# aayush9400/3D-Condtional-Stable-Diffusion

Hardware: AMD Instinct MI355X
Metric: latent volumes/sec at 32^3x8ch T=1000 DDPM (higher is better)
Workload: dtype f32 (f16 hi+lo x3 MFMA, f32 accumulate)

## Files before the change

### 3d-condtional-stable-diffusion_amd/csrc/dm3d_conv_h3w.hip

```cpp
#include <cstdlib>
#include "dm3d_conv_h3v2_parts.h"

using namespace h3v2;

#ifdef DM3D_CLOCK_STAMPS
__device__ unsigned long long* g_dbg_stamps_w = nullptr;
extern "C" int dm3d_debug_set_stamps_wino(void* p) { return (int)hipMemcpyToSymbol(HIP_SYMBOL(g_dbg_stamps_w), &p, sizeof(p)); }
#ifndef STAMP_MASK
#define STAMP_MASK 0xffffffffu
#endif
#define STAMP(i) do { if (((STAMP_MASK >> (i)) & 1u) && g_dbg_stamps_w && wave == 0 && __builtin_amdgcn_mbcnt_lo(~0u, 0u) == 0u && cur.ntile == 0 && cur.khalf == 0 && item / ny < 4096u) { \
    g_dbg_stamps_w[(item / ny) * 32 + (i)] = __builtin_amdgcn_s_memtime(); \
    if ((i) == 1) g_dbg_stamps_w[(item / ny) * 32 + 30] = __builtin_amdgcn_s_memrealtime(); \
    if ((i) == 28) g_dbg_stamps_w[(item / ny) * 32 + 31] = __builtin_amdgcn_s_memrealtime(); } } while (0)
#else
#define STAMP(i) do { } while (0)
#endif

namespace {

template <int N, int I = 0, class F>
__device__ __forceinline__ void static_for(F&& f) {
    if constexpr (I < N) {
        f(std::integral_constant<int, I>{});
        static_for<N, I + 1>(f);
    }
}

constexpr int pass_of(int s) { return 3 * s - (s + 1) / 5; }

template <int MODE>
__global__ __launch_bounds__(256, 1) void conv3d_igemm_h3w(const ConvArgs p) {
    constexpr int TD = 8, TH = 8, TW = 8, CK = 16, NT = 64, NW = 4;
    constexpr int HD = TD + 2, HH = TH + 2, HROWS = HD * HH;
    constexpr int RREC = 17;
    constexpr int NS = 20;
    constexpr int WPAIR = 2 * NT * REC;
    constexpr int RING = 4;
    constexpr int WSLOT = WPAIR * 2 / 1024 / NW;
    constexpr int NLD = 5;
    constexpr bool pro = MODE == 1, xh2 = MODE == 2;
    constexpr int PLOADS = pro ? 4 : 0;

    extern __shared__ __attribute__((aligned(16))) _Float16 smem_w[];
    _Float16* lds_w = smem_w;
    _Float16* lds_in = smem_w + RING * WPAIR;

    const int tid = threadIdx.x;
    const int lane = tid & 63, wave = __builtin_amdgcn_readfirstlane(tid >> 6);

    const int ntiles = p.coutpad / NT;
    const unsigned ny = (unsigned)(ntiles * p.ksplit);
    const int bpv = p.bd * p.bh * p.bw;
    const int cpp = p.nchunks / p.ksplit;
    unsigned item, item_end, item_step;
    {
        const unsigned n_items = (unsigned)(p.batch * bpv) * ny, G = gridDim.x, d = blockIdx.x;
        if ((G & 7u) == 0 && (n_items & 7u) == 0) {
            const unsigned per = n_items >> 3;
            item = (d & 7u) * per + (d >> 3); item_end = (d & 7u) * per + per; item_step = G >> 3;
        } else { item = d; item_end = n_items; item_step = G; }
    }
    struct Item { int b, oz0, oy0, ox0, ntile, khalf; };
    auto decode = [&](unsigned w) {
        Item it;
        unsigned brick = w / ny;
        const unsigned by = w - brick * ny;
        it.ntile = (int)(by % (unsigned)ntiles); it.khalf = (int)(by / (unsigned)ntiles);
        it.b = (int)(brick / (unsigned)bpv);
        brick -= (unsigned)(it.b * bpv);
        it.oz0 = (int)(brick / (unsigned)(p.bh * p.bw)) * TD;
        it.oy0 = (int)((brick / (unsigned)p.bw) % (unsigned)p.bh) * TH;
        it.ox0 = (int)(brick % (unsigned)p.bw) * TW;
        it.b = __builtin_amdgcn_readfirstlane(it.b); it.oz0 = __builtin_amdgcn_readfirstlane(it.oz0); it.oy0 = __builtin_amdgcn_readfirstlane(it.oy0);
        it.ox0 = __builtin_amdgcn_readfirstlane(it.ox0); it.ntile = __builtin_amdgcn_readfirstlane(it.ntile); it.khalf = __builtin_amdgcn_readfirstlane(it.khalf);
        return it;
    };
    Item cur = decode(item);
    auto vec_row = [&](const Item& it) { return p.vec ? (p.vec_idx ? p.vec_idx[it.b] : it.b) : 0; };
    int vrow_s = vec_row(cur);
    int c_lo = cur.khalf * cpp, c_hi = c_lo + cpp;
    STAMP(0);

    int piece = 0;
    bool s_act = false;
    unsigned st_addr = 0u, a_pair[2] = {0u, 0u}, wb_hi = 0u;
    int w_voff = 0;
    constexpr int DZB = HH * RREC * REC * 2, DYB = RREC * REC * 2;
    const unsigned in_addr = (unsigned)(size_t)(__attribute__((address_space(3))) _Float16*)lds_in;
    const unsigned w_addr = (unsigned)(size_t)(__attribute__((address_space(3))) _Float16*)lds_w;
    auto lane_setup = [&]() {
        int t = tid;
        asm volatile("" : "+v"(t));
        const int ln = t & 63, half = ln >> 5, q = (ln >> 4) & 1, row = ln & 15;
        piece = t & 1;
        s_act = (t >> 1) < HROWS;
        const int srow = s_act ? (t >> 1) : HROWS - 1;
        st_addr = in_addr + (unsigned)(srow * RREC * REC + ((piece ^ ((srow % HH) & 2)) << 3)) * 2u;
        const int ay = row & 3, xq = (row >> 2) ^ (row >> 3);
        const unsigned a_base = in_addr + (unsigned)((((2 * wave) * HH + ay) * RREC + xq) * (REC * 2));
        unsigned sl[3];
#pragma unroll
        for (int dy = 0; dy < 3; ++dy) sl[dy] = (unsigned)((q ^ ((ay + dy) & 2)) << 4);
        a_pair[0] = a_base + (half ? DYB + sl[1] : sl[0]);
        a_pair[1] = a_base + 2 * DYB + sl[2] + (half ? DZB : 0);
        const int b_pos = pi_pos(row);
        wb_hi = w_addr + (unsigned)((half * NT + b_pos) * REC + ((q ^ swz(b_pos)) << 3)) * 2u;
        w_voff = wave * 1024 + ln * 16;
    };
    lane_setup();
    int sb, gv0;
    bool row_in, x_lo, x_hi;
    auto stage_setup = [&](const Item& it) {
        int tid_s = tid;
        asm volatile("" : "+v"(tid_s));
        const int sr = (tid_s >> 1) < HROWS ? (tid_s >> 1) : HROWS - 1, hz = sr / HH, hy = sr % HH;
        const int iz = it.oz0 - 1 + hz, iy = it.oy0 - 1 + hy;
        row_in = iz >= 0 && iz < p.ind && iy >= 0 && iy < p.inh;
        x_lo = it.ox0 > 0; x_hi = it.ox0 + TW < p.inw;
        const int izc = iz < 0 ? 0 : (iz >= p.ind ? p.ind - 1 : iz), iyc = iy < 0 ? 0 : (iy >= p.inh ? p.inh - 1 : iy);
        gv0 = ((it.b * p.ind + izc) * p.inh + iyc) * p.inw + it.ox0 - 1;
        sb = it.b;
    };
    stage_setup(cur);
    f32x4v acc[4][4][4];

    const auto w_rsrc = __builtin_amdgcn_make_buffer_rsrc(const_cast<void*>(p.wpk), (short)0, (int)((long)ntiles * p.nchunks * (NS * WPAIR * 2)), 0x00020000);
    auto w_chunk = [&](int ntile_, int ch_) { return (unsigned)((ntile_ * p.nchunks + ch_) * (NS * WPAIR * 2)); };
    unsigned w_cur = w_chunk(cur.ntile, c_lo), w_nxt = w_cur;
    auto fetch_w1 = [&](const unsigned off, int slot, const int i) {
        char* dst = reinterpret_cast<char*>(lds_w) + slot * (WPAIR * 2) + wave * 1024;
        __builtin_amdgcn_raw_ptr_buffer_load_lds(w_rsrc, (__attribute__((address_space(3))) void*)(dst + i * (NW * 1024)), 16, w_voff,
                                                 (int)(off + i * (NW * 1024)), 0, 0);
    };
#pragma unroll
    for (int i = 0; i < RING; ++i) { fetch_w1(w_cur + i * (WPAIR * 2), i, 0); fetch_w1(w_cur + i * (WPAIR * 2), i, 1); }

    f32x4 va[10][2];
    u32x4 oh[4], ol[4];
    u32x4 o3h[4], o3l[4];
    f32x4 sc0 = {1.f, 1.f, 1.f, 1.f}, sc1 = sc0, sh0 = {0.f, 0.f, 0.f, 0.f}, sh1 = sh0;
    bool km[3][2] = {{true, true}, {true, true}, {true, true}};
    bool ok0 = true, ok1 = true;
    auto load_voxel = [&](int ch, int hx) {
        const int hxc = hx == 0 ? (x_lo ? 0 : 1) : (hx == 9 ? (x_hi ? 9 : 8) : hx);
        const unsigned gv = (unsigned)(gv0 + hxc);
        if (xh2) {
            const char* base = reinterpret_cast<const char*>(p.x1) + (size_t)ch * 64;
            const unsigned off = gv * ((unsigned)p.c1 * 4u) + (unsigned)piece * 16u;
            va[hx][0] = *reinterpret_cast<const f32x4*>(base + off);
            va[hx][1] = *reinterpret_cast<const f32x4*>(base + off + 32u);
            return;
        }
        const int c0 = ch * CK;
        const float* src;
        int ldc, cb;
        if (c0 < p.c1) { src = p.x1; ldc = p.c1; cb = c0; } else { src = p.x2; ldc = p.c2; cb = c0 - p.c1; }
        const int cpos = cb + piece * 8;
        const int off0 = cpos < ldc ? cpos : 0, off1 = cpos + 4 < ldc ? cpos + 4 : 0;
        const char* base = reinterpret_cast<const char*>(src);
        const unsigned voff = gv * ((unsigned)ldc * 4u);
        va[hx][0] = *reinterpret_cast<const f32x4*>(base + (voff + (unsigned)off0 * 4u));
        va[hx][1] = *reinterpret_cast<const f32x4*>(base + (voff + (unsigned)off1 * 4u));
    };
    auto load_chunk_params = [&](int ch) {
        if (xh2) return;
        const int c0 = ch * CK;
        const int ldc = c0 < p.c1 ? p.c1 : p.c2, cpos = (c0 < p.c1 ? c0 : c0 - p.c1) + piece * 8;
        ok0 = cpos < ldc;
        ok1 = cpos + 4 < ldc;
        if (pro) {
            const int s0 = ok0 ? c0 + piece * 8 : 0, s1 = ok1 ? c0 + piece * 8 + 4 : 0;
            const size_t bo = (size_t)sb * p.pro_bstride;
            sc0 = *reinterpret_cast<const f32x4*>(p.pscale + bo + s0);
            sh0 = *reinterpret_cast<const f32x4*>(p.pshift + bo + s0);
            sc1 = *reinterpret_cast<const f32x4*>(p.pscale + bo + s1);
            sh1 = *reinterpret_cast<const f32x4*>(p.pshift + bo + s1);
        }
    };
    auto halo_ops = [&](int s) {
        if (s < 0) s += NS;
        if (s >= NLD) return 0;
        return 4 + (s == 0 ? PLOADS : 0);
    };
    typedef float f32x2 __attribute__((ext_vector_type(2)));
    h8 g_hi, g_lo;
#define DM3D_PIN(x) asm volatile("" :: "v"(x))
    auto act_quad = [&](const int hx, const int h) {
        const int col = hx == 0 ? 0 : (hx == 9 ? 2 : 1);
        f32x4 v;
        if (xh2) {
            if (h == 0) { g_hi = __builtin_bit_cast(h8, va[hx][0]); g_lo = __builtin_bit_cast(h8, va[hx][1]); }
#pragma unroll
            for (int e = 0; e < 4; ++e) { const _Float16 a = g_hi[4 * h + e], b = g_lo[4 * h + e]; v[e] = (float)a + (float)b; }
            if (!km[col][0]) v = f32x4{0.f, 0.f, 0.f, 0.f};
        } else {
            v = va[hx][h];
            if (pro) {
                const f32x4 y = __builtin_elementwise_fma(v, h ? sc1 : sc0, h ? sh1 : sh0);
                const f32x4 z = y * -1.4426950408889634f;
                f32x4 d;
#pragma unroll
                for (int e = 0; e < 4; ++e) d[e] = __builtin_amdgcn_exp2f(z[e]);
                d = d + 1.0f;
#pragma unroll
                for (int e = 0; e < 4; ++e) d[e] = __builtin_amdgcn_rcpf(d[e]);
                v = y * d;
            }
            if (!km[col][h]) v = f32x4{0.f, 0.f, 0.f, 0.f};
        }
        DM3D_PIN(v);
        va[hx][h] = v;
    };
    auto split_pair = [&](const int t, const int xt, const int j) {
        const int h = j >> 1, c = 2 * (j & 1);
        auto d = [&](const int k) { return f32x2{va[2 * xt + k][h][c], va[2 * xt + k][h][c + 1]}; };
        const f32x2 x = t == 0 ? d(0) - d(2) : (t == 1 ? d(1) + d(2) : (t == 2 ? d(2) - d(1) : d(1) - d(3)));
        const float x0 = x[0], x1 = x[1];
        unsigned int a, r;
        float r0, r1;
        asm volatile("v_cvt_pk_f16_f32 %0, %4, %5\n\tv_fma_mix_f32 %2, %0, -1.0, %4 op_sel_hi:[1,0,0]\n\t"
                     "v_fma_mix_f32 %3, %0, -1.0, %5 op_sel:[1,0,0] op_sel_hi:[1,0,0]\n\tv_cvt_pk_f16_f32 %1, %2, %3"
                     : "=&v"(a), "=&v"(r), "=&v"(r0), "=&v"(r1) : "v"(x0), "v"(x1));
        if (t == 3) { o3h[xt][j] = a; o3l[xt][j] = r; } else { oh[xt][j] = a; ol[xt][j] = r; }
    };
    auto chunk_masks = [&]() {
        km[0][0] = row_in && x_lo && ok0; km[0][1] = row_in && x_lo && ok1; km[1][0] = row_in && ok0; km[1][1] = row_in && ok1;
        km[2][0] = row_in && x_hi && ok0; km[2][1] = row_in && x_hi && ok1;
    };
    auto store_record = [&](const int t, const int xt) {
        if (s_act) {
            unsigned lo_addr;
            const u32x4 dh = t == 3 ? o3h[xt] : oh[xt], dl = t == 3 ? o3l[xt] : ol[xt];
            switch (t * 4 + xt) {
#define DM3D_ST(k_) case k_: asm volatile("ds_write_b128 %1, %2 offset:%4\n\tv_xor_b32 %0, 32, %1\n\tds_write_b128 %0, %3 offset:%4" \
                                          : "=&v"(lo_addr) : "v"(st_addr), "v"(dh), "v"(dl), "n"((k_) * REC * 2) : "memory"); break;
                DM3D_ST(0) DM3D_ST(1) DM3D_ST(2) DM3D_ST(3) DM3D_ST(4) DM3D_ST(5) DM3D_ST(6) DM3D_ST(7)
                DM3D_ST(8) DM3D_ST(9) DM3D_ST(10) DM3D_ST(11) DM3D_ST(12) DM3D_ST(13) DM3D_ST(14) DM3D_ST(15)
#undef DM3D_ST
            }
        }
    };
    auto lds_barrier = [&]() {
        asm volatile("s_waitcnt lgkmcnt(0)" ::: "memory");
        __builtin_amdgcn_s_barrier();
        asm volatile("" ::: "memory");
    };

#pragma unroll
    for (int hx = 0; hx < 10; ++hx) load_voxel(c_lo, hx);
    load_chunk_params(c_lo);
#pragma unroll
    for (int t = 0; t < 4; ++t)
#pragma unroll
        for (int pi = 0; pi < 4; ++pi)
#pragma unroll
            for (int ni = 0; ni < 4; ++ni) {
                acc[t][pi][ni] = f32x4v{0.f, 0.f, 0.f, 0.f};
                asm volatile("" : "+a"(acc[t][pi][ni]));
            }
    __builtin_amdgcn_s_waitcnt(0x0F70);
    chunk_masks();
#pragma unroll
    for (int hx = 0; hx < 10; ++hx) { act_quad(hx, 0); act_quad(hx, 1); }
#pragma unroll
    for (int t = 0; t < 4; ++t) {
#pragma unroll
        for (int u = 0; u < 16; ++u) split_pair(t, u >> 2, u & 3);
#pragma unroll
        for (int xt = 0; xt < 4; ++xt) store_record(t, xt);
    }
    lds_barrier();

    h8 ah[4], al[4], bh[4], bl[4];
    auto lo_of = [](const unsigned a) { unsigned r; asm volatile("v_xor_b32 %0, 32, %1" : "=v"(r) : "v"(a)); return r; };
#define DM3D_DSR(dst, addr, off) asm volatile("ds_read_b128 %0, %1 offset:%2" : "=v"(dst) : "v"(addr), "n"(off))
    constexpr int GOFF = 4 * RREC * REC * 2, SOFF = HH * RREC * REC * 2;
    auto a_hi = [&](const int s) { return a_pair[(s % 5) >= 3]; };
    auto read_a = [&](h8 (&dst)[4], const int s, const int i, const unsigned a0) {
        const int tp = s % 5;
        switch (((s / 5) * 4 + i) * 3 + (tp < 3 ? tp : tp - 3)) {
#define DM3D_RA1(t_, i_, z_) case ((t_) * 4 + (i_)) * 3 + (z_): DM3D_DSR(dst[i_], a0, (z_) * DZB + (t_) * 4 * REC * 2 + ((i_) >> 1) * SOFF + ((i_) & 1) * GOFF); break;
#define DM3D_RA(t_, i_) DM3D_RA1(t_, i_, 0) DM3D_RA1(t_, i_, 1) DM3D_RA1(t_, i_, 2)
            DM3D_RA(0, 0) DM3D_RA(0, 1) DM3D_RA(0, 2) DM3D_RA(0, 3) DM3D_RA(1, 0) DM3D_RA(1, 1) DM3D_RA(1, 2) DM3D_RA(1, 3)
            DM3D_RA(2, 0) DM3D_RA(2, 1) DM3D_RA(2, 2) DM3D_RA(2, 3) DM3D_RA(3, 0) DM3D_RA(3, 1) DM3D_RA(3, 2) DM3D_RA(3, 3)
#undef DM3D_RA
#undef DM3D_RA1
        }
    };
    auto read_b = [&](h8 (&dst)[4], const int slot, const int i, const unsigned wa) {
        switch (slot * 4 + i) {
#define DM3D_RB(k_, i_) case (k_) * 4 + (i_): DM3D_DSR(dst[i_], wa, (k_) * WPAIR * 2 + (i_) * 16 * REC * 2); break;
            DM3D_RB(0, 0) DM3D_RB(0, 1) DM3D_RB(0, 2) DM3D_RB(0, 3) DM3D_RB(1, 0) DM3D_RB(1, 1) DM3D_RB(1, 2) DM3D_RB(1, 3)
            DM3D_RB(2, 0) DM3D_RB(2, 1) DM3D_RB(2, 2) DM3D_RB(2, 3) DM3D_RB(3, 0) DM3D_RB(3, 1) DM3D_RB(3, 2) DM3D_RB(3, 3)
#undef DM3D_RB
        }
    };
    f32x4 g_y, g_z;
    float g_x0 = 0.f, g_x1 = 0.f, g_r0 = 0.f;
    unsigned int g_a = 0u;
    constexpr int NPASS = 3 * NS - NS / 5;
    auto stores_at_head = [&](int p) {
        p = (p + NPASS) % NPASS;
        if (p == 36 || p == 37 || p == 39 || p == 40 || p == 42 || p == 43) return 2;
        if (p == 38 || p == 41 || p == 44) return 4;
        return p == 54 ? 8 : 0;
    };
    auto head_stores = [&](const int p) {
        if (p == 36) store_record(0, 0); else if (p == 37) store_record(0, 1); else if (p == 38) { store_record(0, 2); store_record(0, 3); }
        else if (p == 39) store_record(1, 0); else if (p == 40) store_record(1, 1); else if (p == 41) { store_record(1, 2); store_record(1, 3); }
        else if (p == 42) store_record(2, 0); else if (p == 43) store_record(2, 1); else if (p == 44) { store_record(2, 2); store_record(2, 3); }
        else if (p == 54) {
#pragma unroll
            for (int xt = 0; xt < 4; ++xt) store_record(3, xt);
        }
    };
    auto slot_gap = [&](const int G) {
        if (G == 191) { chunk_masks(); return; }
        if (G >= 192 && G < 552) {
            const int i = (G - 192) / 18, r = (G - 192) % 18;
            const int hx = i >> 1, h = i & 1, col = hx == 0 ? 0 : (hx == 9 ? 2 : 1);
            if (xh2) {
                auto mix = [&](const int c) {
                    float d;
                    const float hv = va[hx][0][c >> 1], lv = va[hx][1][c >> 1];
                    if (c & 1) asm volatile("v_fma_mix_f32 %0, %1, 1.0, %2 op_sel:[1,0,1] op_sel_hi:[1,0,1]" : "=v"(d) : "v"(hv), "v"(lv));
                    else asm volatile("v_fma_mix_f32 %0, %1, 1.0, %2 op_sel:[0,0,0] op_sel_hi:[1,0,1]" : "=v"(d) : "v"(hv), "v"(lv));
                    return d;
                };
                if (h == 0) {
                    if (r < 2) { g_y[2 * r] = mix(2 * r); g_y[2 * r + 1] = mix(2 * r + 1); }
                } else {
                    if (r < 2) {
                        const float v0 = mix(4 + 2 * r), v1 = mix(5 + 2 * r);
                        va[hx][1][2 * r] = v0; va[hx][1][2 * r + 1] = v1;
                    } else if (r < 4) {
                        const int c = 2 * (r - 2);
                        float v0 = km[col][0] ? g_y[c] : 0.0f, v1 = km[col][0] ? g_y[c + 1] : 0.0f;
                        DM3D_PIN(v0); DM3D_PIN(v1);
                        va[hx][0][c] = v0; va[hx][0][c + 1] = v1;
                    } else if (r < 6) {
                        const int c = 2 * (r - 4);
                        float v0 = km[col][0] ? va[hx][1][c] : 0.0f, v1 = km[col][0] ? va[hx][1][c + 1] : 0.0f;
                        DM3D_PIN(v0); DM3D_PIN(v1);
                        va[hx][1][c] = v0; va[hx][1][c + 1] = v1;
                    }
                }
                return;
            }
            if (!pro) {
                if (r < 2) {
                    const int c = 2 * r;
                    float v0 = km[col][h] ? va[hx][h][c] : 0.0f, v1 = km[col][h] ? va[hx][h][c + 1] : 0.0f;
                    DM3D_PIN(v0); DM3D_PIN(v1);
                    va[hx][h][c] = v0; va[hx][h][c + 1] = v1;
                }
                return;
            }
            const f32x4 sc = h ? sc1 : sc0, sh = h ? sh1 : sh0;
            if (r < 2) {
                const int c = 2 * r;
                g_y[c] = fmaf(va[hx][h][c], sc[c], sh[c]); g_y[c + 1] = fmaf(va[hx][h][c + 1], sc[c + 1], sh[c + 1]);
                DM3D_PIN(g_y[c]); DM3D_PIN(g_y[c + 1]);
            } else if (r < 4) {
                const int c = 2 * (r - 2);
                g_z[c] = g_y[c] * -1.4426950408889634f; g_z[c + 1] = g_y[c + 1] * -1.4426950408889634f;
                DM3D_PIN(g_z[c]); DM3D_PIN(g_z[c + 1]);
            } else if (r < 8) {
                g_z[r - 4] = __builtin_amdgcn_exp2f(g_z[r - 4]);
                DM3D_PIN(g_z[r - 4]);
            } else if (r < 10) {
                const int c = 2 * (r - 8);
                g_z[c] = 1.0f + g_z[c]; g_z[c + 1] = 1.0f + g_z[c + 1];
                DM3D_PIN(g_z[c]); DM3D_PIN(g_z[c + 1]);
            } else if (r < 14) {
                g_z[r - 10] = __builtin_amdgcn_rcpf(g_z[r - 10]);
                DM3D_PIN(g_z[r - 10]);
            } else if (r < 16) {
                const int c = 2 * (r - 14);
                g_y[c] = g_y[c] * g_z[c]; g_y[c + 1] = g_y[c + 1] * g_z[c + 1];
                DM3D_PIN(g_y[c]); DM3D_PIN(g_y[c + 1]);
            } else {
                const int c = 2 * (r - 16);
                float v0 = km[col][h] ? g_y[c] : 0.0f, v1 = km[col][h] ? g_y[c + 1] : 0.0f;
                DM3D_PIN(v0); DM3D_PIN(v1);
                va[hx][h][c] = v0; va[hx][h][c + 1] = v1;
            }
            return;
        }
        if ((G >= 560 && G < 704) || (G >= 816 && G < 864)) {
            const int t = G < 608 ? 0 : (G < 656 ? 1 : (G < 704 ? 2 : 3));
            const int q = G - (t == 0 ? 560 : (t == 1 ? 608 : (t == 2 ? 656 : 816)));
            const int u = q / 3, st = q % 3, xt = u >> 2, j = u & 3, h = j >> 1, c = 2 * (j & 1);
            if (st == 0) {
                auto d = [&](const int k, const int e) { return va[2 * xt + k][h][c + e]; };
                g_x0 = t == 0 ? d(0, 0) - d(2, 0) : (t == 1 ? d(1, 0) + d(2, 0) : (t == 2 ? d(2, 0) - d(1, 0) : d(1, 0) - d(3, 0)));
                g_x1 = t == 0 ? d(0, 1) - d(2, 1) : (t == 1 ? d(1, 1) + d(2, 1) : (t == 2 ? d(2, 1) - d(1, 1) : d(1, 1) - d(3, 1)));
                DM3D_PIN(g_x0); DM3D_PIN(g_x1);
            } else if (st == 1) {
                asm volatile("v_cvt_pk_f16_f32 %0, %2, %3\n\tv_fma_mix_f32 %1, %0, -1.0, %2 op_sel_hi:[1,0,0]" : "=&v"(g_a), "=&v"(g_r0) : "v"(g_x0), "v"(g_x1));
            } else {
                unsigned int r;
                float r1;
                asm volatile("v_fma_mix_f32 %1, %2, -1.0, %3 op_sel:[1,0,0] op_sel_hi:[1,0,0]\n\tv_cvt_pk_f16_f32 %0, %4, %1" : "=&v"(r), "=&v"(r1) : "v"(g_a), "v"(g_x1), "v"(g_r0));
                if (t == 3) { o3h[xt][j] = g_a; o3l[xt][j] = r; } else { oh[xt][j] = g_a; ol[xt][j] = r; }
            }
        }
    };
#define DM3D_MFMA(T, PI, NI, A, B) asm volatile("v_mfma_f32_16x16x32_f16 %0, %1, %2, %0" : "+a"(acc[T][PI][NI]) : "v"(A[PI]), "v"(B[NI]))
#define DM3D_WAIT_LGKM(n) asm volatile("s_waitcnt lgkmcnt(%0)" :: "n"(n) : "memory")

    bool has_next = item + item_step < item_end;
    for (;;) {
    lane_setup();
    {
        const unsigned a_lo0 = lo_of(a_hi(0));
        read_a(al, 0, 0, a_lo0); read_a(al, 0, 1, a_lo0); read_a(al, 0, 2, a_lo0); read_a(al, 0, 3, a_lo0);
    }
    read_b(bh, 0, 0, wb_hi); read_b(bh, 0, 1, wb_hi); read_b(bh, 0, 2, wb_hi); read_b(bh, 0, 3, wb_hi);
    read_a(ah, 0, 0, a_hi(0)); read_a(ah, 0, 1, a_hi(0)); read_a(ah, 0, 2, a_hi(0)); read_a(ah, 0, 3, a_hi(0));
    STAMP(1);

    for (int ch = c_lo; ch < c_hi; ++ch) {
        asm volatile("" : "+v"(gv0));
        int ch_next;
        if (ch + 1 < c_hi) { ch_next = ch + 1; w_nxt = w_cur + NS * WPAIR * 2; }
        else if (has_next) {
            const Item n = decode(item + item_step);
            stage_setup(n); ch_next = n.khalf * cpp; w_nxt = w_chunk(n.ntile, ch_next);
        }
        else { ch_next = ch; w_nxt = w_cur; }
        static_for<NS>([&](auto S_) {
            constexpr int s = decltype(S_)::value, sn = (s + 1) % NS;
            constexpr int t = s / 5, ws = s & (RING - 1), ws1 = (s + 1) & (RING - 1);
            constexpr bool pad = s % 5 == 3, pre_pad = s % 5 == 2, post_pad = s % 5 == 4;
            constexpr int E = pass_of(s);
            constexpr bool swapped = (((s + 1) / 5) & 1) != 0;
            h8 (&fh)[4] = swapped ? al : ah;
            h8 (&fl)[4] = swapped ? ah : al;
            h8 (&fl_n)[4] = pad ? fh : fl;
            h8 (&fh_n)[4] = pad ? fl : fh;
            {
                constexpr int n_out = pad ? 0 : 4;
                switch (post_pad ? 0 : stores_at_head(E - 1)) {
                case 0: DM3D_WAIT_LGKM(n_out); break;
                case 2: DM3D_WAIT_LGKM(n_out + 2); break;
                case 4: DM3D_WAIT_LGKM(n_out + 4); break;
                default: DM3D_WAIT_LGKM(n_out + 8); break;
                }
            }
            head_stores(E);
            __builtin_amdgcn_sched_barrier(0);
            unsigned b_lo = 0u, a_lo = 0u;
#pragma unroll
            for (int g = 0; g < 16; ++g) {
                DM3D_MFMA(t, g >> 2, g & 3, fl, bh);
                slot_gap(16 * E + g);
                if (g == 2) b_lo = lo_of(wb_hi);
                if (g == 3) { read_b(bl, ws, 0, b_lo); read_b(bl, ws, 1, b_lo); }
                if (pre_pad) {
                    if (g == 4) asm volatile("v_subrev_u32 %0, %2, %1" : "=v"(a_lo) : "v"(a_pair[1]), "n"(DZB));
                    if (g == 5) asm volatile("v_xor_b32 %0, 32, %0" : "+v"(a_lo));
                    if (g == 6) asm volatile("v_cndmask_b32_e64 %0, %1, %0, %2" : "+v"(a_lo) : "v"(a_pair[1]), "s"(0xffffffff00000000ull));
                } else if (g == 6) a_lo = lo_of(a_hi(sn));
                if (g == 7) { read_b(bl, ws, 2, b_lo); read_b(bl, ws, 3, b_lo); read_a(fl_n, sn, 0, a_lo); }
                if (g == 11) { read_a(fl_n, sn, 1, a_lo); read_a(fl_n, sn, 2, a_lo); }
                if (g == 15) read_a(fl_n, sn, 3, a_lo);
                __builtin_amdgcn_sched_barrier(0);
            }
            {
                constexpr int DMA_BEHIND = 2 * WSLOT;
                const int extra = halo_ops(s - 3) + halo_ops(s - 2) + halo_ops(s - 1);
#define DM3D_WAIT_VM_LGKM4(n) __builtin_amdgcn_s_waitcnt((((n) & 15) | (7 << 4) | (4 << 8) | ((((n) >> 4) & 3) << 14)))
                switch (extra) {
                case 0:  DM3D_WAIT_VM_LGKM4(DMA_BEHIND); break;
                case 4:  DM3D_WAIT_VM_LGKM4(DMA_BEHIND + 4); break;
                case 8:  DM3D_WAIT_VM_LGKM4(DMA_BEHIND + 8); break;
                case 12: DM3D_WAIT_VM_LGKM4(DMA_BEHIND + 12); break;
                case 16: DM3D_WAIT_VM_LGKM4(DMA_BEHIND + 16); break;
                default: DM3D_WAIT_VM_LGKM4(0); break;
                }
#undef DM3D_WAIT_VM_LGKM4
                __builtin_amdgcn_s_barrier();
                asm volatile("" ::: "memory");
            }
            __builtin_amdgcn_sched_barrier(0);
            const unsigned w_src = s + RING < NS ? w_cur + (s + RING) * (WPAIR * 2) : w_nxt + (s + RING - NS) * (WPAIR * 2);
            fetch_w1(w_src, ws, 0);
            head_stores(E + 1);
            __builtin_amdgcn_sched_barrier(0);
#pragma unroll
            for (int g = 0; g < 16; ++g) {
                if (pad) {
                    DM3D_MFMA(t, g >> 2, g & 3, fl, bl);
                    slot_gap(16 * (E + 1) + g);
                    if (g == 2) { read_b(bh, ws1, 0, wb_hi); read_b(bh, ws1, 1, wb_hi); }
                    if (g == 3) { read_b(bh, ws1, 2, wb_hi); read_b(bh, ws1, 3, wb_hi); }
                    if (g == 4) read_a(fh_n, sn, 0, a_hi(sn));
                    if (g == 7 || g == 11 || g == 15) read_a(fh_n, sn, g >> 2, a_hi(sn));
                } else {
                    DM3D_MFMA(t, g & 3, g >> 2, fh, bh);
                    slot_gap(16 * (E + 1) + g);
                    if ((g & 3) == 3) read_b(bh, ws1, g >> 2, wb_hi);
                }
                if (g == 1) fetch_w1(w_src, ws, 1);
                if (s < NLD && g == 5) load_voxel(ch_next, 2 * s);
                if (s < NLD && g == 9) load_voxel(ch_next, 2 * s + 1);
                if (s == 0 && g == 13) load_chunk_params(ch_next);
                __builtin_amdgcn_sched_barrier(0);
            }
            if constexpr (!pad) {
                head_stores(E + 2);
                __builtin_amdgcn_sched_barrier(0);
#pragma unroll
                for (int g = 0; g < 16; ++g) {
                    DM3D_MFMA(t, g >> 2, g & 3, fh, bl);
                    slot_gap(16 * (E + 2) + g);
                    if (!pre_pad && (g & 3) == 3) read_a(fh, sn, g >> 2, a_hi(sn));
                    __builtin_amdgcn_sched_barrier(0);
                }
            }
        });
        w_cur = w_nxt;
    }
#undef DM3D_MFMA
#undef DM3D_WAIT_LGKM
#undef DM3D_PIN
#undef DM3D_DSR
    STAMP(28);
    const Brick br = {cur.b, cur.oz0, cur.oy0, cur.ox0, p.ooz, p.ooy, p.oox, cur.ntile, cur.khalf};
    {
        asm volatile("s_waitcnt lgkmcnt(0)" ::: "memory");
        STAMP(20);
        const bool skip = p.s_npairs > 0;
        if (skip) {
#pragma unroll
            for (int pi = 0; pi < 4; ++pi)
#pragma unroll
                for (int ni = 0; ni < 4; ++ni) {
                    const f32x4v m0 = acc[0][pi][ni], m1 = acc[1][pi][ni], m2 = acc[2][pi][ni], m3 = acc[3][pi][ni];
                    acc[0][pi][ni] = (m0 + m1) + m2;
                    acc[1][pi][ni] = (m1 - m2) - m3;
                    asm volatile("" : "+a"(acc[0][pi][ni]), "+a"(acc[1][pi][ni]));
                }
            const int p_lo = p.s_npairs * cur.khalf / p.ksplit, np = p.s_npairs * (cur.khalf + 1) / p.ksplit;
            int lane_t = lane;
            asm volatile("" : "+v"(lane_t));
            const int kq = lane_t >> 4, lhalf = kq >> 1, cq = (kq & 1) * 8, row_t = lane_t & 15;
            unsigned sv[8];
#pragma unroll
            for (int t = 0; t < 8; ++t) {
                const int z = 2 * wave + (t >> 2), y = 4 * ((t >> 1) & 1) + (row_t & 3), x = 2 * ((row_t >> 2) ^ (row_t >> 3)) + (t & 1);
                sv[t] = (unsigned)(((cur.b * p.ind + cur.oz0 + z) * p.inh + cur.oy0 + y) * p.inw + cur.ox0 + x);
            }
            const char* swf = reinterpret_cast<const char*>(p.swpk_f) + (size_t)cur.ntile * p.s_npairs * 8192 + lane_t * 16;
            f32x4 ar0[2][8], ar1[2][8];
            h8 bw[2][8];
            float lim0[2], lim1[2];
            auto t_load = [&](auto SET, int pp) {
                constexpr int S = decltype(SET)::value;
                const int c0 = (pp * 2 + lhalf) * CK;
                const float* src;
                int ldc, cb;
                if (c0 < p.sc1) { src = p.sx1; ldc = p.sc1; cb = c0; } else { src = p.sx2; ldc = p.sc2; cb = c0 - p.sc1; }
                const int cpos = cb + cq;
                const bool real = src != nullptr && cb < ldc && pp < np;
                const bool k0 = real && cpos < ldc, k1 = real && cpos + 4 < ldc;
                lim0[S] = k0 ? 65504.0f : 0.0f;
                lim1[S] = k1 ? 65504.0f : 0.0f;
                const char* base = reinterpret_cast<const char*>(real ? src : p.sx1);
                const unsigned ld4 = (unsigned)(real ? ldc : p.sc1) * 4u, o0 = (unsigned)(k0 ? cpos : 0) * 4u, o1 = (unsigned)(k1 ? cpos + 4 : 0) * 4u;
#pragma unroll
                for (int t = 0; t < 8; ++t) {
                    ar0[S][t] = *reinterpret_cast<const f32x4*>(base + (sv[t] * ld4 + o0));
                    ar1[S][t] = *reinterpret_cast<const f32x4*>(base + (sv[t] * ld4 + o1));
                }
                const char* ws = swf + (size_t)(pp < p.s_npairs ? pp : p.s_npairs - 1) * 8192;
#pragma unroll
                for (int f = 0; f < 8; ++f) bw[S][f] = *reinterpret_cast<const h8*>(ws + f * 1024);
            };
#define DM3D_TMFMA(ACC, A, B) asm volatile("v_mfma_f32_16x16x32_f16 %0, %1, %2, %0" : "+a"(ACC) : "v"(A), "v"(B))
            auto t_step = [&](auto SET) {
                constexpr int S = decltype(SET)::value;
                h8 ahi[8], alo[8];
#pragma unroll
                for (int t = 0; t < 8; ++t) split8(ar0[S][t], ar1[S][t], lim0[S], lim1[S], ahi[t], alo[t]);
                __builtin_amdgcn_sched_barrier(0);
                asm volatile("s_nop 1" ::: "memory");
                __builtin_amdgcn_sched_barrier(0);
#pragma unroll
                for (int t = 0; t < 8; ++t)
#pragma unroll
                    for (int ni = 0; ni < 4; ++ni) DM3D_TMFMA(acc[t & 1][t >> 1][ni], alo[t], bw[S][2 * ni]);
#pragma unroll
                for (int t = 0; t < 8; ++t)
#pragma unroll
                    for (int ni = 0; ni < 4; ++ni) DM3D_TMFMA(acc[t & 1][t >> 1][ni], ahi[t], bw[S][2 * ni + 1]);
#pragma unroll
                for (int t = 0; t < 8; ++t)
#pragma unroll
                    for (int ni = 0; ni < 4; ++ni) DM3D_TMFMA(acc[t & 1][t >> 1][ni], ahi[t], bw[S][2 * ni]);
            };
#undef DM3D_TMFMA
            const std::integral_constant<int, 0> S0;
            const std::integral_constant<int, 1> S1;
            t_load(S0, p_lo);
            for (int pp = p_lo; pp < np; pp += 2) {
                t_load(S1, pp + 1);
                t_step(S0);
                t_load(S0, pp + 2);
                t_step(S1);
            }
            asm volatile("s_nop 7\n\ts_nop 7" ::: "memory");
        }
        auto slice_tiles = [&](auto S_, f32x4v (&e)[4][4]) {
            constexpr int s = decltype(S_)::value;
#pragma unroll
            for (int t = 0; t < 4; ++t)
#pragma unroll
                for (int g = 0; g < 2; ++g)
#pragma unroll
                    for (int ni = 0; ni < 4; ++ni) asm volatile("" : "+a"(acc[t][2 * s + g][ni]));
            if (skip) {
#pragma unroll
                for (int g = 0; g < 2; ++g)
#pragma unroll
                    for (int ni = 0; ni < 4; ++ni) { e[2 * g][ni] = acc[0][2 * s + g][ni]; e[2 * g + 1][ni] = acc[1][2 * s + g][ni]; }
            } else {
#pragma unroll
                for (int g = 0; g < 2; ++g)
#pragma unroll
                    for (int ni = 0; ni < 4; ++ni) {
                        const f32x4v m0 = acc[0][2 * s + g][ni], m1 = acc[1][2 * s + g][ni], m2 = acc[2][2 * s + g][ni], m3 = acc[3][2 * s + g][ni];
                        e[2 * g][ni] = (m0 + m1) + m2;
                        e[2 * g + 1][ni] = (m1 - m2) - m3;
                    }
            }
        };
        bool finish = true;
        const long tile = (long)(item / ny) * ntiles + cur.ntile;
        SplitTile stile = {};
        if (p.ksplit > 1) {
            stile = split_tile(p, tile, cur.khalf);
            static_for<2>([&](auto S_) {
                __builtin_amdgcn_sched_barrier(0);
                f32x4v e[4][4];
                slice_tiles(S_, e);
                split_store(stile, e, 16 * decltype(S_)::value);
            });
            finish = split_is_last(p, tile, reinterpret_cast<unsigned*>(lds_in + HROWS * RREC * REC));
        }
        if (finish) {
            float gn[8];
            const EpiVecs ev = epilogue_cq_vecs(p, br, vrow_s);
#pragma unroll
            for (int i = 0; i < 8; ++i) gn[i] = 0.0f;
            static_for<2>([&](auto S_) {
                constexpr int s = decltype(S_)::value;
                __builtin_amdgcn_sched_barrier(0);
                if (s == 1) STAMP(21);
                f32x4v e[4][4];
                slice_tiles(S_, e);
                if (p.ksplit > 1) split_gather(stile, p, cur.khalf, e, 16 * s);
#ifndef DM3D_EXP_NO_EPILOGUE
                epilogue_cq<TD>(p, e, br, 2 * wave + s, ev, vrow_s, p.gn_stats ? gn : nullptr);
#else
                if (e[0][0][0] == 12345.678f) p.out[0] = e[1][1][1] + e[2][2][2] + e[3][3][3];
#endif
            });
            if (p.gn_stats) gn_flush_cq<TD>(p, gn, br, 2 * wave, 2);
        }
        STAMP(29);
        if (!has_next) break;
        __builtin_amdgcn_sched_barrier(0);
#pragma unroll
        for (int t = 0; t < 4; ++t)
#pragma unroll
            for (int pi = 0; pi < 4; ++pi)
#pragma unroll
                for (int ni = 0; ni < 4; ++ni) {
                    acc[t][pi][ni] = f32x4v{0.f, 0.f, 0.f, 0.f};
                    asm volatile("" : "+a"(acc[t][pi][ni]));
                }
        item += item_step;
        cur = decode(item);
        vrow_s = vec_row(cur);
        c_lo = cur.khalf * cpp; c_hi = c_lo + cpp;
        has_next = item + item_step < item_end;
    }
    }
}

template <int MODE>
int launch_w(const ConvLaunch& r, hipStream_t st) {
    constexpr size_t lds = (size_t)(4 * 2 * 64 * REC + 10 * 10 * 17 * REC) * sizeof(_Float16) + 16;
    static_assert(lds <= 160 * 1024, "one workgroup per CU");
    static std::atomic<bool> attr_set[64] = {};
    static std::atomic<int> cus[64] = {};
    const int dev = dm3d_dyn_lds(lds, attr_set, "conv", &conv3d_igemm_h3w<MODE>);
    if (dev < 0) return dev;
    if (cus[dev].load(std::memory_order_acquire) == 0) {
        int n = 0;
        DM3D_HIP(hipDeviceGetAttribute(&n, hipDeviceAttributeMultiprocessorCount, dev));
        cus[dev].store(n > 0 ? n : 256, std::memory_order_release);
    }
    const int ncu = cus[dev].load(std::memory_order_relaxed);
    H3v2Launch L;
    if (int rc = dm3d_h3v2_pre_launch(r, L)) return rc;
    ConvArgs& k = L.k;
    k.wpk = k.wpk_wino;
    const long items = (long)k.batch * k.bd * k.bh * k.bw * (k.coutpad / 64) * k.ksplit;
    static const bool persist = [] { const char* e = getenv("DM3D_CONV_WINO_PERSIST"); return !(e && e[0] == '0'); }();
    long g = items;
    if (persist && items > ncu) g = (items % 8 == 0 && ncu >= 8) ? (ncu / 8 * 8) : ncu;
    if (g < 1) g = 1;
    if (persist) {
        const char* cap = getenv("DM3D_CONV_WINO_GRID");
        if (cap && atol(cap) > 0 && atol(cap) < g) g = atol(cap);
    }
    hipLaunchKernelGGL((conv3d_igemm_h3w<MODE>), dim3((unsigned)g), dim3(256), lds, st, k);
    if (int rc = dm3d_launch_check("conv3d_igemm_h3w")) return rc;
    return dm3d_h3v2_post_launch(r.a, L, st);
}

}

int dm3d_conv_launch_h3w(const ConvLaunch& r, hipStream_t st) {
    if (r.a.x_h2) return launch_w<2>(r, st);
    return r.a.pscale ? launch_w<1>(r, st) : launch_w<0>(r, st);
}
```

Before: 2.399.

## Pair weight slots into a 3-granule ring and barrier only every other stage

Reorganizes the LDS weight ring from four single-stage slots into three double-stage granules, with a rotating set of slot offsets and a prefetch distance of five stages. The workgroup barrier and vmem wait now run only on odd stages, and even stages do just an lgkm wait. The B-read base address advances per granule. This halves the barriers per chunk and deepens weight prefetch, at the cost of more LDS for weights, rotating offset registers, and a reshuffled head-store schedule.

Result: no change. 2.413 (median of 6 runs) (+0.6%).

```diff
diff --git a/3d-condtional-stable-diffusion_amd/csrc/dm3d_conv_h3w.hip b/3d-condtional-stable-diffusion_amd/csrc/dm3d_conv_h3w.hip
--- a/3d-condtional-stable-diffusion_amd/csrc/dm3d_conv_h3w.hip
+++ b/3d-condtional-stable-diffusion_amd/csrc/dm3d_conv_h3w.hip
@@ -36,7 +36,9 @@
     constexpr int RREC = 17;
     constexpr int NS = 20;
     constexpr int WPAIR = 2 * NT * REC;
-    constexpr int RING = 4;
+    constexpr int WGRAN = 2 * WPAIR;
+    constexpr int RING = 3;
+    constexpr int WAHEAD = 5;
     constexpr int WSLOT = WPAIR * 2 / 1024 / NW;
     constexpr int NLD = 5;
     constexpr bool pro = MODE == 1, xh2 = MODE == 2;
@@ -44,7 +46,7 @@
 
     extern __shared__ __attribute__((aligned(16))) _Float16 smem_w[];
     _Float16* lds_w = smem_w;
-    _Float16* lds_in = smem_w + RING * WPAIR;
+    _Float16* lds_in = smem_w + RING * WGRAN;
 
     const int tid = threadIdx.x;
     const int lane = tid & 63, wave = __builtin_amdgcn_readfirstlane(tid >> 6);
@@ -89,6 +91,7 @@
     constexpr int DZB = HH * RREC * REC * 2, DYB = RREC * REC * 2;
     const unsigned in_addr = (unsigned)(size_t)(__attribute__((address_space(3))) _Float16*)lds_in;
     const unsigned w_addr = (unsigned)(size_t)(__attribute__((address_space(3))) _Float16*)lds_w;
+    unsigned so0 = 0u, so1 = (unsigned)(WGRAN * 2), so2 = (unsigned)(2 * WGRAN * 2);
     auto lane_setup = [&]() {
         int t = tid;
         asm volatile("" : "+v"(t));
@@ -105,7 +108,7 @@
         a_pair[0] = a_base + (half ? DYB + sl[1] : sl[0]);
         a_pair[1] = a_base + 2 * DYB + sl[2] + (half ? DZB : 0);
         const int b_pos = pi_pos(row);
-        wb_hi = w_addr + (unsigned)((half * NT + b_pos) * REC + ((q ^ swz(b_pos)) << 3)) * 2u;
+        wb_hi = w_addr + so0 + (unsigned)((half * NT + b_pos) * REC + ((q ^ swz(b_pos)) << 3)) * 2u;
         w_voff = wave * 1024 + ln * 16;
     };
     lane_setup();
@@ -128,13 +131,13 @@
     const auto w_rsrc = __builtin_amdgcn_make_buffer_rsrc(const_cast<void*>(p.wpk), (short)0, (int)((long)ntiles * p.nchunks * (NS * WPAIR * 2)), 0x00020000);
     auto w_chunk = [&](int ntile_, int ch_) { return (unsigned)((ntile_ * p.nchunks + ch_) * (NS * WPAIR * 2)); };
     unsigned w_cur = w_chunk(cur.ntile, c_lo), w_nxt = w_cur;
-    auto fetch_w1 = [&](const unsigned off, int slot, const int i) {
-        char* dst = reinterpret_cast<char*>(lds_w) + slot * (WPAIR * 2) + wave * 1024;
+    auto fetch_w1 = [&](const unsigned off, const unsigned dst_off, const int i) {
+        char* dst = reinterpret_cast<char*>(lds_w) + dst_off + wave * 1024;
         __builtin_amdgcn_raw_ptr_buffer_load_lds(w_rsrc, (__attribute__((address_space(3))) void*)(dst + i * (NW * 1024)), 16, w_voff,
                                                  (int)(off + i * (NW * 1024)), 0, 0);
     };
 #pragma unroll
-    for (int i = 0; i < RING; ++i) { fetch_w1(w_cur + i * (WPAIR * 2), i, 0); fetch_w1(w_cur + i * (WPAIR * 2), i, 1); }
+    for (int i = 0; i < WAHEAD; ++i) { fetch_w1(w_cur + i * (WPAIR * 2), (unsigned)(i * (WPAIR * 2)), 0); fetch_w1(w_cur + i * (WPAIR * 2), (unsigned)(i * (WPAIR * 2)), 1); }
 
     f32x4 va[10][2];
     u32x4 oh[4], ol[4];
@@ -288,11 +291,11 @@
 #undef DM3D_RA1
         }
     };
+    auto so = [&](const int k) { return k % RING == 0 ? so0 : (k % RING == 1 ? so1 : so2); };
     auto read_b = [&](h8 (&dst)[4], const int slot, const int i, const unsigned wa) {
         switch (slot * 4 + i) {
 #define DM3D_RB(k_, i_) case (k_) * 4 + (i_): DM3D_DSR(dst[i_], wa, (k_) * WPAIR * 2 + (i_) * 16 * REC * 2); break;
             DM3D_RB(0, 0) DM3D_RB(0, 1) DM3D_RB(0, 2) DM3D_RB(0, 3) DM3D_RB(1, 0) DM3D_RB(1, 1) DM3D_RB(1, 2) DM3D_RB(1, 3)
-            DM3D_RB(2, 0) DM3D_RB(2, 1) DM3D_RB(2, 2) DM3D_RB(2, 3) DM3D_RB(3, 0) DM3D_RB(3, 1) DM3D_RB(3, 2) DM3D_RB(3, 3)
 #undef DM3D_RB
         }
     };
@@ -302,14 +305,14 @@
     constexpr int NPASS = 3 * NS - NS / 5;
     auto stores_at_head = [&](int p) {
         p = (p + NPASS) % NPASS;
-        if (p == 36 || p == 37 || p == 39 || p == 40 || p == 42 || p == 43) return 2;
-        if (p == 38 || p == 41 || p == 44) return 4;
+        if (p == 36 || p == 37 || p == 39 || p == 40) return 2;
+        if (p == 38 || p == 41 || p == 43 || p == 44) return 4;
         return p == 54 ? 8 : 0;
     };
     auto head_stores = [&](const int p) {
         if (p == 36) store_record(0, 0); else if (p == 37) store_record(0, 1); else if (p == 38) { store_record(0, 2); store_record(0, 3); }
         else if (p == 39) store_record(1, 0); else if (p == 40) store_record(1, 1); else if (p == 41) { store_record(1, 2); store_record(1, 3); }
-        else if (p == 42) store_record(2, 0); else if (p == 43) store_record(2, 1); else if (p == 44) { store_record(2, 2); store_record(2, 3); }
+        else if (p == 43) { store_record(2, 0); store_record(2, 1); } else if (p == 44) { store_record(2, 2); store_record(2, 3); }
         else if (p == 54) {
 #pragma unroll
             for (int xt = 0; xt < 4; ++xt) store_record(3, xt);
@@ -432,7 +435,8 @@
         else { ch_next = ch; w_nxt = w_cur; }
         static_for<NS>([&](auto S_) {
             constexpr int s = decltype(S_)::value, sn = (s + 1) % NS;
-            constexpr int t = s / 5, ws = s & (RING - 1), ws1 = (s + 1) & (RING - 1);
+            constexpr int t = s / 5, ws = s & 1, ws1 = (s + 1) & 1;
+            constexpr bool odd = (s & 1) != 0;
             constexpr bool pad = s % 5 == 3, pre_pad = s % 5 == 2, post_pad = s % 5 == 4;
             constexpr int E = pass_of(s);
             constexpr bool swapped = (((s + 1) / 5) & 1) != 0;
@@ -464,11 +468,12 @@
                     if (g == 6) asm volatile("v_cndmask_b32_e64 %0, %1, %0, %2" : "+v"(a_lo) : "v"(a_pair[1]), "s"(0xffffffff00000000ull));
                 } else if (g == 6) a_lo = lo_of(a_hi(sn));
                 if (g == 7) { read_b(bl, ws, 2, b_lo); read_b(bl, ws, 3, b_lo); read_a(fl_n, sn, 0, a_lo); }
+                if (odd && g == 9) { wb_hi += so((s + 1) / 2) - so((s - 1) / 2); DM3D_PIN(wb_hi); }
                 if (g == 11) { read_a(fl_n, sn, 1, a_lo); read_a(fl_n, sn, 2, a_lo); }
                 if (g == 15) read_a(fl_n, sn, 3, a_lo);
                 __builtin_amdgcn_sched_barrier(0);
             }
-            {
+            if constexpr (odd) {
                 constexpr int DMA_BEHIND = 2 * WSLOT;
                 const int extra = halo_ops(s - 3) + halo_ops(s - 2) + halo_ops(s - 1);
 #define DM3D_WAIT_VM_LGKM4(n) __builtin_amdgcn_s_waitcnt((((n) & 15) | (7 << 4) | (4 << 8) | ((((n) >> 4) & 3) << 14)))
@@ -483,10 +488,14 @@
 #undef DM3D_WAIT_VM_LGKM4
                 __builtin_amdgcn_s_barrier();
                 asm volatile("" ::: "memory");
+            } else {
+                __builtin_amdgcn_s_waitcnt(15 | (7 << 4) | (4 << 8) | (3 << 14));
             }
             __builtin_amdgcn_sched_barrier(0);
-            const unsigned w_src = s + RING < NS ? w_cur + (s + RING) * (WPAIR * 2) : w_nxt + (s + RING - NS) * (WPAIR * 2);
-            fetch_w1(w_src, ws, 0);
+            constexpr int sq = s + WAHEAD;
+            const unsigned w_src = sq < NS ? w_cur + sq * (WPAIR * 2) : w_nxt + (sq - NS) * (WPAIR * 2);
+            const unsigned w_dst = so(sq / 2) + (unsigned)((sq & 1) * (WPAIR * 2));
+            fetch_w1(w_src, w_dst, 0);
             head_stores(E + 1);
             __builtin_amdgcn_sched_barrier(0);
 #pragma unroll
@@ -503,7 +512,7 @@
                     slot_gap(16 * (E + 1) + g);
                     if ((g & 3) == 3) read_b(bh, ws1, g >> 2, wb_hi);
                 }
-                if (g == 1) fetch_w1(w_src, ws, 1);
+                if (g == 1) fetch_w1(w_src, w_dst, 1);
                 if (s < NLD && g == 5) load_voxel(ch_next, 2 * s);
                 if (s < NLD && g == 9) load_voxel(ch_next, 2 * s + 1);
                 if (s == 0 && g == 13) load_chunk_params(ch_next);
@@ -522,6 +531,7 @@
             }
         });
         w_cur = w_nxt;
+        { const unsigned o = so0; so0 = so1; so1 = so2; so2 = o; }
     }
 #undef DM3D_MFMA
 #undef DM3D_WAIT_LGKM
@@ -693,7 +703,7 @@
 
 template <int MODE>
 int launch_w(const ConvLaunch& r, hipStream_t st) {
-    constexpr size_t lds = (size_t)(4 * 2 * 64 * REC + 10 * 10 * 17 * REC) * sizeof(_Float16) + 16;
+    constexpr size_t lds = (size_t)(3 * 2 * 2 * 64 * REC + 10 * 10 * 17 * REC) * sizeof(_Float16) + 16;
     static_assert(lds <= 160 * 1024, "one workgroup per CU");
     static std::atomic<bool> attr_set[64] = {};
     static std::atomic<int> cus[64] = {};
```
